# funkelab/cellulus

Hardware: AMD Instinct MI355X
Metric: train crops/sec (U-Net fwd+bwd + OCE loss + Adam) (higher is better)
Workload: dtype f32 (exact 3xbf16 operand split, 6 products, f32 accumulate)

## Files before the change

### cellulus_amd/_clx.py

```python

import ctypes
import os
from ctypes import POINTER, Structure, c_char_p, c_double, c_int, c_longlong, c_size_t, c_void_p

import torch

_HERE = os.path.dirname(os.path.abspath(__file__))
LIB_PATH = os.path.join(_HERE, "libclx.so")


class ClxError(RuntimeError):
    """A libclx entry point returned a negative status."""


class ClxSrc(Structure):

    _fields_ = [
        ("ptr", c_void_p),
        ("C", c_int),
        ("ld", c_int),
        ("D", c_int),
        ("H", c_int),
        ("W", c_int),
        ("oz", c_int),
# ... 52 lines not shown
        ("ld_pool", c_int),
        ("tile_list", c_void_p),
        ("tile_count", c_int),
        ("precision", c_int),
        ("wplanes", c_void_p),
        ("aplanes", c_void_p),
        ("aplanes_valid", c_int),
        ("dyplanes", c_void_p),
        ("dyplanes_valid", c_int),
        ("out_planes", c_void_p),
        ("out_colsum", c_void_p),
    ]


_P = c_void_p
_I = c_int
_LL = c_longlong
_D = c_double

PROTOTYPES = {
    "clx_last_error": (c_char_p, []),
    "clx_abi_version": (_I, []),
    "clx_device_count": (_I, []),
    "clx_profile_enable": (_I, [_I]),
    "clx_profile_read": (_I, [_I, POINTER(c_double), POINTER(c_double), POINTER(c_double)]),
    "clx_profile_clock": (_I, [POINTER(c_double), POINTER(c_double), _I]),
    "clx_conv_fwd": (_I, [POINTER(ClxConvDesc), _P]),
    "clx_conv_wgrad": (_I, [POINTER(ClxConvDesc), _P, _I, _P, _P, _P]),
    "clx_chain64_fwd": (_I, [_P, _I, _LL, _P, _P, _P, _I, _P, _I, _P, _P, _I, _I, _P, _I, _P, _I, _P]),
    "clx_chain64_bwd": (_I, [_P, _I, _I, _P, _I, _P, _I, _I, _LL, _P, _P, _P, _I, _P, _P, _P, _P, _P]),
    "clx_pack_weights": (_I, [_P, _P, _I, _I, _I, _I, _I, _I, _P]),
    "clx_pack_weights_batch": (_I, [_P, _I, _LL, _P]),
    "clx_unpack_wgrad": (_I, [_P, _P, _I, _I, _I, _I, _I, _P]),
    "clx_unpack_wgrad_wino": (_I, [_P, _P, _I, _I, _I, _I, _I, _I, _I, _P]),
    "clx_conv_workspace_bytes": (c_size_t, [POINTER(ClxConvDesc), _I]),
    "clx_conv_vcache_bytes": (c_size_t, [POINTER(ClxConvDesc), _I]),
    "clx_conv_sp_covers": (_I, [POINTER(ClxConvDesc), _I]),
    "clx_planes_bytes": (c_size_t, [_LL, _I]),
    "clx_split_planes": (_I, [_P, _LL, _LL, _I, _P, _P]),
    "clx_join_planes": (_I, [_P, _LL, _I, _P, _LL, _P]),
    "clx_gemm_planes": (_I, [_P, _P, _I, _I, _I, _P, _I, _P, _I, _P]),
    "clx_wgrad_planes": (_I, [_P, _P, _LL, _I, _I, _P, _I, _P]),
    "clx_conv_fused_applicable": (_I, [POINTER(ClxConvDesc)]),
    "clx_conv_fused_workspace_bytes": (c_size_t, [POINTER(ClxConvDesc)]),
    "clx_planar_to_pixel": (_I, [_P, _P, _I, _I, _LL, _I, _P]),
    "clx_pixel_to_planar": (_I, [_P, _P, _I, _I, _LL, _I, _P]),
# ... 169 lines not shown
```

### cellulus_amd/csrc/clx_common.h

```cpp
#pragma once
#include <hip/hip_runtime.h>
#include <hip/hip_ext.h>
#include <stdint.h>
#include <stdio.h>
#include <stdarg.h>
#include "../../include/clx.h"

void clx_set_error(const char* fmt, ...);

#define CLX_REQUIRE(cond, ...)                \
  do {                                        \
    if (!(cond)) {                            \
      clx_set_error(__VA_ARGS__);             \
      return CLX_ERR_ARG;                     \
    }                                         \
  } while (0)

#define CLX_CHECK_LAUNCH(name)                                           \
  do {                                                                   \
    hipError_t e__ = hipGetLastError();                                  \
    if (e__ != hipSuccess) {                                             \
      clx_set_error("%s: launch failed: %s", name, hipGetErrorString(e__)); \
      return CLX_ERR_LAUNCH;                                             \
    }                                                                    \
// ... 7 lines not shown
};
static inline FastDiv make_fastdiv(uint32_t d) {
  FastDiv f;
  f.d = d;
  uint32_t l = 0;
  while ((1ull << l) < d) ++l;
  f.l = l;
  f.m = (uint32_t)(((1ull << 32) * ((1ull << l) - d)) / d + 1);
  return f;
}
__device__ __forceinline__ uint32_t fdiv(uint32_t n, const FastDiv& f) {
  return (__umulhi(f.m, n) + n) >> f.l;
}

__device__ __forceinline__ int xcd_remap(int bid, int nblocks) {
  const int q = nblocks >> 3, r = nblocks & 7;
  const int xcd = bid & 7, idx = bid >> 3;
  const int base = (xcd < r) ? xcd * (q + 1) : r * (q + 1) + (xcd - r) * q;
  return base + idx;
}

static inline int cdiv(long long a, long long b) { return (int)((a + b - 1) / b); }

int clx_conv_validate(const clx_conv_desc* d, const char* who);

bool clx_smallc_applicable(const clx_conv_desc* d);
int clx_smallc_fwd(const clx_conv_desc* d, hipStream_t st);
int clx_smallc_wgrad(const clx_conv_desc* d, const float* dy, int ld_dy, float* dwpack,
                     float* dbias, hipStream_t st);

int clx_igemm_launch(const clx_conv_desc* d, int batch, long long bs_in, long long bs_w,
                     long long bs_out, hipStream_t st);
int clx_wgrad_launch(const clx_conv_desc* d, const float* dy, int ld_dy, float* dwpack, float* dbias,
                     int batch, long long bs_x, long long bs_dy, long long bs_out, hipStream_t st);
bool clx_sp_fwd_rule(const clx_conv_desc* d);
bool clx_sp_wgrad_rule(const clx_conv_desc* d);
bool clx_sp_applicable(const clx_conv_desc* d);
bool clx_wino_sp(const clx_conv_desc* d);
int clx_sp_launch(const void* A, const void* B, int M, int N, int K, long long rows_a, int batch, long long bs_a, long long bs_b,
                  long long bs_out, const clx_conv_desc* ep, hipStream_t st);
int clx_sp_clock_read(double* shader_ticks, double* wall_ticks, int reset);
int clx_sp_split(const float* x, long long ld, long long rows, int K, void* planes, float* colsum, int nreal, hipStream_t st);
int clx_sp_wgrad_launch(const void* dy_planes, const void* x_planes, long long rows, int N, int C, int batch, long long bs_dy,
                        long long bs_x, long long bs_out, float* dw, int ld_dw, hipStream_t st);
int clx_wino_fwd(const clx_conv_desc* d, hipStream_t st);
int clx_wino_wgrad(const clx_conv_desc* d, const float* dy, int ld_dy, float* dwpack, float* dbias,
// ... 17 lines not shown
```

### cellulus_amd/csrc/clx_core.hip

```cpp
#include "clx_common.h"

static thread_local char g_err[512] = "";

void clx_set_error(const char* fmt, ...) {
  va_list ap;
  va_start(ap, fmt);
  vsnprintf(g_err, sizeof(g_err), fmt, ap);
  va_end(ap);
}

extern "C" const char* clx_last_error(void) { return g_err; }
extern "C" int clx_abi_version(void) { return 13; }
extern "C" int clx_device_count(void) {
  int n = 0;
  if (hipGetDeviceCount(&n) != hipSuccess) {
    (void)hipGetLastError();
    return 0;
  }
  return n;
}

#include <vector>

namespace {
struct ProfRec { int kind; double flops; hipEvent_t e0, e1; };
bool g_prof_on = false;
std::vector<ProfRec> g_prof;
}

bool clx_prof_enabled() { return g_prof_on; }

void clx_prof_events(int kind, double flops, hipEvent_t* e0, hipEvent_t* e1) {
  *e0 = *e1 = nullptr;
  ProfRec r;
  r.kind = kind; r.flops = flops;
  if (hipEventCreate(&r.e0) != hipSuccess) return;
  if (hipEventCreate(&r.e1) != hipSuccess) { (void)hipEventDestroy(r.e0); return; }
  g_prof.push_back(r);
  *e0 = r.e0; *e1 = r.e1;
}

extern "C" int clx_profile_enable(int on) {
  g_prof_on = on != 0;
// ... 20 lines not shown
```

### cellulus_amd/csrc/conv_smallc.hip

```cpp
#include "clx_common.h"

namespace {

struct SmallP {
  const float* x;
  int ld_x, B, D, H, W;
  int oz, oy, ox;
  int ID, IH, IW, KD, KH, KW, PD, PH, PW, OD, OH, OW;
  int N, M, taps;
  FastDiv dOW, dOH, dOD;
  const float* wpack;
  const float* bias;
  float* out;
  int ld_out, relu;
  const float* dy;
  int ld_dy;
  float* dwp;
  float* dbias;
  int tiles_per_block;
  int RX, items;
  FastDiv dRX;
};

constexpr int PT = 64;
// ... 388 lines not shown
    f32x4 acc = bv;
#pragma unroll
    for (int rr = 0; rr < R; ++rr)
#pragma unroll
      for (int tx = 0; tx < 3; ++tx) acc += xv[rr * 3 + tx] * w[rr * 3 + tx];
    if (relu) {
#pragma unroll
      for (int e = 0; e < 4; ++e) acc[e] = fmaxf(acc[e], 0.f);
    }
    if (live && live_n) *reinterpret_cast<f32x4*>(out + (size_t)r * ld_out + nn) = acc;
  }
}

bool grey_applicable(const clx_conv_desc* d, int ld_act) {
  return d->c_real == 1 && d->KH == 3 && d->KW == 3 && (d->KD == 1 || d->KD == 3) && d->PD == 0 &&
         d->PH == 0 && d->PW == 0 && d->N % 4 == 0 && ld_act % 4 == 0;
}

dim3 grey_grid(SmallP& p) {
  p.RX = cdiv(p.OW, 4);
  p.items = p.B * p.OD * p.OH * p.RX;
  p.dRX = make_fastdiv(p.RX);
  const int ny = cdiv(p.N, 64);
  int nx = 768 / ny;
  if (nx < 1) nx = 1;
  if (nx > cdiv(p.items, 4)) nx = cdiv(p.items, 4);
  return dim3(nx, ny);
}

bool fill(const clx_conv_desc* d, SmallP& p) {
  const clx_src& S = d->src[0];
  p.x = S.ptr; p.ld_x = S.ld; p.B = d->B; p.D = S.D; p.H = S.H; p.W = S.W;
  p.oz = S.oz; p.oy = S.oy; p.ox = S.ox;
  p.ID = d->ID; p.IH = d->IH; p.IW = d->IW;
  p.KD = d->KD; p.KH = d->KH; p.KW = d->KW;
  p.PD = d->PD; p.PH = d->PH; p.PW = d->PW;
  p.OD = d->ID + 2 * d->PD - d->KD + 1;
  p.OH = d->IH + 2 * d->PH - d->KH + 1;
  p.OW = d->IW + 2 * d->PW - d->KW + 1;
  p.N = d->N;
  p.M = d->B * p.OD * p.OH * p.OW;
  p.taps = d->KD * d->KH * d->KW;
  p.dOW = make_fastdiv(p.OW); p.dOH = make_fastdiv(p.OH); p.dOD = make_fastdiv(p.OD);
  return true;
}

int pick_ng(int N) {
  int ng = 4;
  while (ng < 64 && ng * 4 < N) ng *= 2;
  return ng;
// ... 85 lines not shown
```

### cellulus_amd/csrc/gemm_sp.hip

```cpp
#include "clx_common.h"
#include "sp_planes.h"
#include <stdlib.h>
#include <type_traits>

__device__ unsigned long long g_sp_clk_ticks[2];
int clx_sp_clock_read(double* shader_ticks, double* wall_ticks, int reset) {
  unsigned long long h[2] = {0ull, 0ull};
  if (hipMemcpyFromSymbol(h, HIP_SYMBOL(g_sp_clk_ticks), sizeof(h)) != hipSuccess) return CLX_ERR_LAUNCH;
  *shader_ticks = (double)h[0];
  *wall_ticks = (double)h[1];
  if (reset) {
    const unsigned long long z[2] = {0ull, 0ull};
    if (hipMemcpyToSymbol(HIP_SYMBOL(g_sp_clk_ticks), z, sizeof(z)) != hipSuccess) return CLX_ERR_LAUNCH;
  }
  return CLX_OK;
}

namespace {

typedef __bf16 bf16x8 __attribute__((ext_vector_type(8)));
using sp::u32x2;
using sp::u32x4;
using sp::FRAG;
using sp::KSTEP;
// ... 959 lines not shown
  }
  return cache[dev];
}

int clx_sp_zero_tail(void* planes, long long rows, int K, int batch, long long bs, hipStream_t st) {
  if (sp::padded_rows(rows) == rows || batch <= 0) return CLX_OK;
  const int ksteps = K / 16;
  const long long total = (sp::padded_rows(rows) / 32 - rows / 32) * ksteps * 6 * 32;
  sp_zero_tail_kernel<<<dim3((unsigned)cdiv(total, 256), (unsigned)batch), 256, 0, st>>>((char*)planes, bs, rows, ksteps);
  return CLX_OK;
}

extern "C" size_t clx_planes_bytes(long long rows, int K) {
  if (rows <= 0 || K <= 0 || K % 16 != 0) return 0;
  return (size_t)sp::planes_bytes(rows, K);
}

int clx_sp_split(const float* x, long long ld, long long rows, int K, void* planes, float* colsum, int nreal, hipStream_t st) {
  CLX_REQUIRE(x != nullptr && planes != nullptr, "clx_split_planes: null pointer");
  CLX_REQUIRE(rows > 0 && K > 0 && K % 16 == 0 && ld >= K && ld % 4 == 0, "clx_split_planes: K must be a multiple of 16, ld >= K a multiple of 4");
  CLX_REQUIRE(((uintptr_t)x & 15) == 0 && ((uintptr_t)planes & 15) == 0, "clx_split_planes: pointers must be 16-byte aligned");
  const int ksteps = K / 16;
  const long long nfrag = sp::padded_rows(rows) / 32 * ksteps;
  long long blocks = (nfrag + 3) / 4;
  if (blocks > 8192) blocks = 8192;
  if (colsum != nullptr) {
    if (blocks > 2048) blocks = 2048;
    int g = ksteps % 4 == 0 ? 4 : ksteps % 2 == 0 ? 2 : 1;
    const long long unit = ksteps / g;
    blocks = (blocks + unit - 1) / unit * unit;
    CLX_LAUNCH_KIND(CLX_PROF_SPLIT_PLANES, sp_split_kernel<true>, dim3((unsigned)blocks), dim3(256), 0, st, x, ld, rows, ksteps, (char*)planes,
                    nfrag, colsum, nreal);
  } else {
    CLX_LAUNCH_KIND(CLX_PROF_SPLIT_PLANES, sp_split_kernel<false>, dim3((unsigned)blocks), dim3(256), 0, st, x, ld, rows, ksteps, (char*)planes,
                    nfrag, (float*)nullptr, 0);
  }
  return CLX_OK;
}

extern "C" int clx_split_planes(const float* x, long long ld, long long rows, int K, void* planes, clx_stream stream) {
  const int rc = clx_sp_split(x, ld, rows, K, planes, nullptr, 0, (hipStream_t)stream);
  if (rc) return rc;
  CLX_CHECK_LAUNCH("clx_split_planes");
  return CLX_OK;
}

extern "C" int clx_join_planes(const void* planes, long long rows, int K, float* x, long long ld, clx_stream stream) {
  CLX_REQUIRE(x != nullptr && planes != nullptr, "clx_join_planes: null pointer");
  CLX_REQUIRE(rows > 0 && K > 0 && K % 16 == 0 && ld >= K, "clx_join_planes: K must be a multiple of 16, ld >= K");
  const long long nfrag = sp::padded_rows(rows) / 32 * (K / 16);
  long long blocks = (nfrag + 3) / 4;
  if (blocks > 8192) blocks = 8192;
  sp_join_kernel<<<dim3((unsigned)blocks), dim3(256), 0, (hipStream_t)stream>>>((const char*)planes, ld, rows, K / 16, x, nfrag);
  CLX_CHECK_LAUNCH("clx_join_planes");
  return CLX_OK;
}
// ... 126 lines not shown
```

### cellulus_amd/csrc/glue.hip

```cpp
#include "clx_common.h"

namespace {

inline int grid_for(long long total, int block) {
  long long g = (total + block - 1) / block;
  if (g > 8192) g = 8192;
  if (g < 1) g = 1;
  return (int)g;
}

struct Dec {
  FastDiv c4, w, h, d;
};
inline Dec make_dec(int C4, int W, int H, int D) {
  return Dec{make_fastdiv((uint32_t)C4), make_fastdiv((uint32_t)W), make_fastdiv((uint32_t)H), make_fastdiv((uint32_t)D)};
}
__device__ __forceinline__ void decode(uint32_t i, const Dec& dc, uint32_t& pixel, int& c4, int& x, int& y, int& z, int& b) {
  pixel = fdiv(i, dc.c4);
  c4 = (int)(i - pixel * dc.c4.d);
  const uint32_t q1 = fdiv(pixel, dc.w);
  x = (int)(pixel - q1 * dc.w.d);
  const uint32_t q2 = fdiv(q1, dc.h);
  y = (int)(q1 - q2 * dc.h.d);
  const uint32_t q3 = fdiv(q2, dc.d);
  z = (int)(q2 - q3 * dc.d.d);
  b = (int)q3;
}

__device__ __forceinline__ f32x4 ld4(const float* p) { return *reinterpret_cast<const f32x4*>(p); }
__device__ __forceinline__ void st4(float* p, f32x4 v) { *reinterpret_cast<f32x4*>(p) = v; }

__global__ void maxpool_fwd_kernel(const float* __restrict__ x, float* __restrict__ y,
// ... 434 lines not shown
    noise_inject_kernel<1><<<grid_for((long long)T * n, 256), 256, 0, st>>>(rnd, raw, out, T, n_half, n, p);
  CLX_CHECK_LAUNCH("clx_noise_inject");
  return CLX_OK;
}

extern "C" int clx_zero_many(void* const* buffers, const long long* nbytes, int count, clx_stream stream) {
  CLX_REQUIRE(count >= 0 && (count == 0 || (buffers && nbytes)), "clx_zero_many: bad arguments");
  hipStream_t st = (hipStream_t)stream;
  for (int first = 0; first < count; first += 8) {
    ZeroManyP p;
    p.count = 0;
    p.first16[0] = 0;
    for (int k = first; k < count && k < first + 8; ++k) {
      CLX_REQUIRE(nbytes[k] >= 0 && nbytes[k] % 4 == 0, "clx_zero_many: sizes are multiples of 4 bytes");
      if (nbytes[k] == 0) continue;
      CLX_REQUIRE(buffers[k] && ((uintptr_t)buffers[k] & 15) == 0, "clx_zero_many: buffers are 16-byte aligned");
      const int q = p.count++;
      p.base[q] = (unsigned long long)(uintptr_t)buffers[k];
      p.first16[q + 1] = p.first16[q] + (unsigned long long)nbytes[k] / 16;
      p.tail_words[q] = (unsigned int)(nbytes[k] % 16) / 4;
    }
    if (p.count == 0) continue;
    for (int q = p.count; q < 8; ++q) { p.base[q] = 0; p.first16[q + 1] = p.first16[p.count]; p.tail_words[q] = 0; }
    long long g = (long long)((p.first16[p.count] + 255) / 256);
    g = g < 1 ? 1 : (g > 4096 ? 4096 : g);
    zero_many_kernel<<<(int)g, 256, 0, st>>>(p);
  }
  CLX_CHECK_LAUNCH("clx_zero_many");
  return CLX_OK;
}

extern "C" int clx_gather_rows_f64(const double* src, const int* rows, long long n, int width, double* dst,
                                   clx_stream stream) {
  CLX_REQUIRE(n >= 0 && width > 0 && (n == 0 || (src && rows && dst)), "clx_gather_rows_f64: bad arguments");
  if (n == 0) return CLX_OK;
  gather_rows_f64_kernel<<<grid_for(n * width, 256), 256, 0, (hipStream_t)stream>>>(src, rows, n, width, dst);
  CLX_CHECK_LAUNCH("clx_gather_rows_f64");
  return CLX_OK;
}

static int subpixel_launch(bool to_space, const float* src, float* dst, int ld_lo, int ld_hi, int B,
                           int D, int H, int W, int N, int fz, int fy, int fx, hipStream_t st,
                           const char* who) {
  CLX_REQUIRE(src && dst, "%s: null pointer", who);
  CLX_REQUIRE(B > 0 && D > 0 && H > 0 && W > 0 && N > 0 && N % 4 == 0, "%s: bad extents", who);
  CLX_REQUIRE(fz >= 1 && fy >= 1 && fx >= 1, "%s: bad factors", who);
  CLX_REQUIRE(ld_lo % 4 == 0 && ld_lo >= fz * fy * fx * N && ld_hi % 4 == 0 && ld_hi >= N, "%s: bad strides", who);
  const long long total = (long long)B * D * H * W * fz * fy * fx * (N / 4);
  if (to_space)
// ... 84 lines not shown
```

### cellulus_amd/csrc/pack.hip

```cpp
#include "clx_common.h"

namespace {

__global__ void pack_weights_kernel(const float* __restrict__ w, float* __restrict__ wp,
                                    int cout, int cin, int taps, int cin_pad,
                                    int cout_pad, int mode, long long total) {
  for (long long i = (long long)blockIdx.x * blockDim.x + threadIdx.x; i < total;
       i += (long long)gridDim.x * blockDim.x) {
    float v = 0.f;
    if (mode == CLX_PACK_FWD) {
      const int c = (int)(i % cin_pad);
      const long long t = i / cin_pad;
      const int tap = (int)(t % taps);
      const int n = (int)(t / taps);
      if (c < cin) v = w[((long long)n * cin + c) * taps + tap];
    } else {
      const int n = (int)(i % cout_pad);
      const long long t = i / cout_pad;
      const int tap = (int)(t % taps);
      const int c = (int)(t / taps);
      if (n < cout && c < cin) v = w[((long long)n * cin + c) * taps + (taps - 1 - tap)];
    }
    wp[i] = v;
  }
// ... 85 lines not shown
  for (long long i = (long long)blockIdx.x * blockDim.x + threadIdx.x; i < total;
       i += (long long)gridDim.x * blockDim.x) {
    const int tap = (int)(i % taps);
    const long long t = i / taps;
    const int c = (int)(t % g.cin), n = (int)(t / g.cin);
    if (c < g.C0) {
      gw[i] = g_skip[((long long)n * g.C0 + c) * taps + tap];
      continue;
    }
    const int d = tap / (g.k[1] * g.k[2]), h = (tap / g.k[2]) % g.k[1], x = tap % g.k[2];
    float v = 0.f;
    for (int a0 = 0; a0 < g.f[0]; ++a0)
      for (int a1 = 0; a1 < g.f[1]; ++a1)
        for (int a2 = 0; a2 < g.f[2]; ++a2) {
          const int ph = (a0 * g.f[1] + a1) * g.f[2] + a2;
          const int zt = (sp_low_tap(g.f[0], a0, d) * g.zk[1] + sp_low_tap(g.f[1], a1, h)) * g.zk[2] +
                         sp_low_tap(g.f[2], a2, x);
          v += g_eff[(((long long)ph * g.N + n) * g.C1 + (c - g.C0)) * ztaps + zt];
        }
    gw[i] = v;
  }
}

inline int grid_for(long long total, int block) {
  long long g = (total + block - 1) / block;
  if (g > 4096) g = 4096;
  if (g < 1) g = 1;
  return (int)g;
}

}

extern "C" int clx_pack_weights(const float* w, float* wp, int cout, int cin, int taps,
                                int cin_pad, int cout_pad, int mode, clx_stream stream) {
  CLX_REQUIRE(w && wp, "clx_pack_weights: null pointer");
  CLX_REQUIRE(cout > 0 && cin > 0 && taps > 0, "clx_pack_weights: bad extents");
  CLX_REQUIRE(cin_pad >= cin && cout_pad >= cout && cin_pad % 4 == 0 && cout_pad % 4 == 0,
              "clx_pack_weights: padded extents must be >= real and multiples of 4");
  if (mode == CLX_PACK_WINO4_ADJOINT) {
    CLX_REQUIRE(taps == 9 || taps == 27, "clx_pack_weights: the adjoint form exists for 3x3 and 3x3x3 kernels");
    clx_wino_pack(w, wp, cout, cin, cin_pad, cout_pad, 2, 4, 3, taps == 27 ? 3 : 1, (hipStream_t)stream);
    CLX_CHECK_LAUNCH("clx_pack_weights(winograd adjoint)");
    return CLX_OK;
  }
  if (mode == CLX_PACK_WINO4_FUSED) {
    CLX_REQUIRE((taps == 9 || taps == 4) && cout_pad % 64 == 0 && cin_pad % 8 == 0,
                "clx_pack_weights: the fused Winograd layout exists for 2-D 3x3 / 2x2 kernels with cout_pad %% 64 == 0 and "
                "cin_pad %% 8 == 0");
    clx_wino_pack(w, wp, cout, cin, cin_pad, cout_pad, 3, 4, taps == 9 ? 3 : 2, 1, (hipStream_t)stream);
    CLX_CHECK_LAUNCH("clx_pack_weights(winograd fused)");
    return CLX_OK;
  }
// ... 94 lines not shown
```

### cellulus_amd/csrc/wino.hip

```cpp
#include "clx_common.h"
#include "sp_planes.h"
#include "wino_tables.h"

namespace {

inline int grid_for(long long total, int block) {
  long long g = (total + block - 1) / block;
  if (g > 16384) g = 16384;
  if (g < 1) g = 1;
  return (int)g;
}

__device__ __forceinline__ f32x4 ld4(const float* p) { return *reinterpret_cast<const f32x4*>(p); }
__device__ __forceinline__ void st4(float* p, f32x4 v) { *reinterpret_cast<f32x4*>(p) = v; }

struct Geom {
  int B, SH, SW, oy, ox;
  int ID, SD, oz;
  int IH, IW, P;
  int OH, OW, th, tw;
  long long T;
};

template <int MT, int R, bool PL = false>
__global__ __launch_bounds__(256) void wino_input_kernel(const float* __restrict__ x, int ld_x, int C4, Geom g,
                                                         float* __restrict__ V, long long total,
                                                         const int* __restrict__ tile_list = nullptr, long long Tc = 0,
                                                         long long plane_bytes = 0) {
  using W = WT<MT, R>;
  constexpr int A = W::A;
  const int C = C4 * 4;
  const long long Trows = tile_list ? Tc : g.T;
  const long long plane = Trows * C;
  for (long long i = (long long)blockIdx.x * blockDim.x + threadIdx.x; i < total;
// ... 147 lines not shown
        } else {
          for (int e = 0; e < 4 && n + e < Nreal; ++e) {
            float xv = v[e];
            if (mask) xv = (mask[m * ld_mask + n + e] > 0.f) ? xv : 0.f;
            out[m * ld_out + n + e] = xv;
          }
        }
        if (pool_out) {
          if ((a & 1) == 0 && (cc & 1) == 0) pm[a >> 1][cc >> 1] = v;
          else {
#pragma unroll
            for (int e = 0; e < 4; ++e) pm[a >> 1][cc >> 1][e] = fmaxf(pm[a >> 1][cc >> 1][e], v[e]);
          }
          if ((a & 1) && (cc & 1)) {
            const long long pm_ = ((long long)b * (g.OH >> 1) + (oy >> 1)) * (g.OW >> 1) + (ox >> 1);
            st4(pool_out + pm_ * ld_pool + n, pm[a >> 1][cc >> 1]);
          }
        }
      }
    }
  }
}

constexpr int ADJ_SEG = 8;

__global__ __launch_bounds__(256) void wino_adjoint_output_kernel(const float* __restrict__ Pm, int C4, int Bn, int th,
                                                                  int tw, int IH, int IW, const float* __restrict__ mask,
                                                                  int ld_mask, const unsigned int* __restrict__ mask_bits,
                                                                  int ld_mask_bits, float* __restrict__ out, int ld_out,
                                                                  int Creal, long long total) {
  using W = WT<4, 3>;
  constexpr int A = 6;
  const int C = C4 * 4;
  const int bh = (IH + 3) / 4, bw = (IW + 3) / 4;
  const int nseg = (bh + ADJ_SEG - 1) / ADJ_SEG;
  const long long plane = (long long)Bn * th * tw * C;
  for (long long i = (long long)blockIdx.x * blockDim.x + threadIdx.x; i < total;
       i += (long long)gridDim.x * blockDim.x) {
    const int c = (int)(i % C4) * 4;
    long long t = i / C4;
    const int bx = (int)(t % bw);
    long long q = t / bw;
    const int sg = (int)(q % nseg);
    const int b = (int)(q / nseg);
    const int by0 = sg * ADJ_SEG, by1 = min(by0 + ADJ_SEG, bh);
    f32x4 carry[2][4];
#pragma unroll
    for (int a = 0; a < 2; ++a)
#pragma unroll
      for (int e = 0; e < 4; ++e) carry[a][e] = f32x4{0.f, 0.f, 0.f, 0.f};
    for (int ty = by0 - 1; ty < by1; ++ty) {
      f32x4 d[A][4];
#pragma unroll
      for (int a = 0; a < A; ++a)
#pragma unroll
        for (int e = 0; e < 4; ++e) d[a][e] = f32x4{0.f, 0.f, 0.f, 0.f};
      if (ty >= 0 && ty < th) {
#pragma unroll
        for (int ux = 0; ux < 2; ++ux) {
          const int tx = bx - ux;
          if (tx < 0 || tx >= tw) continue;
          const float* src = Pm + (((long long)b * th + ty) * tw + tx) * C + c;
#pragma unroll
          for (int s2 = 0; s2 < A; ++s2) {
            f32x4 pcol[A], wcol[A];
#pragma unroll
            for (int r = 0; r < A; ++r) pcol[r] = ld4(src + (r * A + s2) * plane);
#pragma unroll
            for (int a = 0; a < A; ++a) {
              f32x4 v = {0.f, 0.f, 0.f, 0.f};
              bool first = true;
#pragma unroll
              for (int r = 0; r < A; ++r) axpy(v, first, W::BT[r][a], pcol[r]);
              wcol[a] = v;
            }
#pragma unroll
            for (int e = 0; e < 4; ++e) {
              if (ux && e >= 2) continue;
              const float coef = ux ? W::BT[s2][4 + (e & 1)] : W::BT[s2][e];
#pragma unroll
              for (int a = 0; a < A; ++a) {
                bool first = false;
                axpy(d[a][e], first, coef, wcol[a]);
              }
            }
          }
        }
      }
      if (ty >= by0) {
#pragma unroll
        for (int a = 0; a < 4; ++a) {
          const int y = 4 * ty + a;
          if (y >= IH) continue;
#pragma unroll
          for (int e = 0; e < 4; ++e) {
            const int x = 4 * bx + e;
            if (x >= IW) continue;
            f32x4 v = d[a][e];
            if (a < 2) v += carry[a][e];
            const long long m = ((long long)b * IH + y) * IW + x;
            if (mask_bits) {
              const unsigned int wbits = mask_bits[m * ld_mask_bits + (c >> 5)] >> (c & 31);
#pragma unroll
              for (int k = 0; k < 4; ++k) v[k] = ((wbits >> k) & 1u) ? v[k] : 0.f;
            }
            if (c + 3 < Creal) {
              if (mask) {
                const f32x4 mk = ld4(mask + m * ld_mask + c);
#pragma unroll
                for (int k = 0; k < 4; ++k) v[k] = (mk[k] > 0.f) ? v[k] : 0.f;
              }
              st4(out + m * ld_out + c, v);
            } else {
              for (int k = 0; k < 4 && c + k < Creal; ++k) {
                float xv = v[k];
                if (mask) xv = (mask[m * ld_mask + c + k] > 0.f) ? xv : 0.f;
                out[m * ld_out + c + k] = xv;
              }
            }
          }
        }
      }
#pragma unroll
      for (int e = 0; e < 4; ++e) { carry[0][e] = d[4][e]; carry[1][e] = d[5][e]; }
    }
  }
}

template <int MT, int R, bool PL = false>
__global__ __launch_bounds__(256) void wino_dy_kernel(const float* __restrict__ dy, int ld_dy, int N4,
                                                      Geom g, float* __restrict__ Md,
                                                      float* __restrict__ dbias, int Nreal,
                                                      long long total, long long plane_bytes = 0) {
  using W = WT<MT, R>;
  constexpr int A = W::A;
  extern __shared__ float bacc[];
  const int N = N4 * 4;
  const long long plane = g.T * N;
  if (dbias) {
    for (int k = threadIdx.x; k < N; k += blockDim.x) bacc[k] = 0.f;
    __syncthreads();
  }
  for (long long i = (long long)blockIdx.x * blockDim.x + threadIdx.x; i < total;
       i += (long long)gridDim.x * blockDim.x) {
    int n;
    long long t;
    if constexpr (PL) {
// ... 442 lines not shown
      int rc = clx_sp_zero_tail(V, gin.T, C, AA, pbV, st);
      if (rc) return rc;
      CLX_LAUNCH_KIND(CLX_PROF_WINO_TRANSFORM, (wino_input_kernel<MT, R, true>), dim3(grid_for(tot_in, 256)), dim3(256), 0, st, S.ptr, S.ld, C / 4,
                      gin, V, tot_in, (const int*)nullptr, 0ll, pbV);
    } else {
      const long long tot_in = gin.T * (C / 4);
      CLX_LAUNCH_KIND(CLX_PROF_WINO_TRANSFORM, (wino_input_kernel<MT, R>), dim3(grid_for(tot_in, 256)), dim3(256), 0, st, S.ptr, S.ld, C / 4, gin, V,
                      tot_in, (const int*)nullptr, 0ll, 0ll);
    }
  }
  if (spx) {
    const int rc = clx_sp_zero_tail(Md, gout.T, N, AA, pbM, st);
    if (rc) return rc;
  }
  if (d->dy_vcache) {
    Geom gd = gout;
    gd.SH = gout.OH; gd.SW = gout.OW; gd.oy = gd.ox = 0;
    gd.ID = gd.SD = out_planes(d); gd.oz = 0;
    gd.IH = gout.OH; gd.IW = gout.OW; gd.P = R - 1;
    gd.OH = gout.OH + R - 1; gd.OW = gout.OW + R - 1;
    gd.th = (gd.OH + MT - 1) / MT; gd.tw = (gd.OW + MT - 1) / MT;
    gd.T = (long long)gd.B * gd.th * gd.tw;
    const long long tot = spx ? sp_items(gd.T, N) : gd.T * (N / 4);
    int blocks = grid_for(tot, 256);
    if (dbias && blocks > 2048) blocks = 2048;
    if (spx) {
      const long long pbD = sp::planes_bytes(gd.T, N);
      const int rc = clx_sp_zero_tail(d->dy_vcache, gd.T, N, AA, pbD, st);
      if (rc) return rc;
      CLX_LAUNCH_KIND(CLX_PROF_WINO_TRANSFORM, (wino_dy_dual_kernel<MT, R, true>), dim3(blocks), dim3(256), (size_t)N * sizeof(float), st, dy, ld_dy,
                      N / 4, gd, gout, (float*)d->dy_vcache, Md, dbias, N, tot, pbD, pbM);
    } else {
      CLX_LAUNCH_KIND(CLX_PROF_WINO_TRANSFORM, (wino_dy_dual_kernel<MT, R>), dim3(blocks), dim3(256), (size_t)N * sizeof(float), st, dy, ld_dy, N / 4,
                      gd, gout, (float*)d->dy_vcache, Md, dbias, N, tot, 0ll, 0ll);
    }
  } else {
    const long long tot_dy = spx ? sp_items(gout.T, N) : gout.T * (N / 4);
    int blocks = grid_for(tot_dy, 256);
    if (blocks > 2048) blocks = 2048;
    if (spx)
      CLX_LAUNCH_KIND(CLX_PROF_WINO_TRANSFORM, (wino_dy_kernel<MT, R, true>), dim3(blocks), dim3(256), (size_t)N * sizeof(float), st, dy, ld_dy, N / 4,
                      gout, Md, dbias, N, tot_dy, pbM);
    else
      CLX_LAUNCH_KIND(CLX_PROF_WINO_TRANSFORM, (wino_dy_kernel<MT, R>), dim3(blocks), dim3(256), (size_t)N * sizeof(float), st, dy, ld_dy, N / 4, gout,
                      Md, dbias, N, tot_dy, 0ll);
  }
  if (spx) {
    CLX_REQUIRE(gin.T == gout.T, "clx_conv_wgrad(winograd): tile counts of input and output differ");
    CLX_REQUIRE(d->det_turns == nullptr, "clx_conv_wgrad: the reproducible mode exists for the float32 precision only");
    const int rc = clx_sp_wgrad_launch(Md, V, gin.T, N, C, AA, pbM, pbV, (long long)N * C, dwpack, C, st);
    if (rc) return rc;
    CLX_CHECK_LAUNCH("clx_conv_wgrad(winograd, split precision)");
    return CLX_OK;
  }
  clx_conv_desc gd = gemm_desc(V, C, d, gin);
  gd.N = N;
  gd.det_turns = d->det_turns;
  const int rc = clx_wgrad_launch(&gd, Md, N, dwpack, nullptr, AA, gin.T * C, gout.T * N,
                                  (long long)d->KD * N * C, st);
  if (rc) return rc;
  CLX_CHECK_LAUNCH("clx_conv_wgrad(winograd)");
  return CLX_OK;
// ... 52 lines not shown
  float* P = (float*)d->workspace;
  float* Mdy = P + (size_t)36 * Tdx * Cp;
  if (spx) {
    CLX_REQUIRE(d->wplanes != nullptr, "clx_conv_fwd(adjoint): precision f32x3bf16 needs wplanes");
    const char* Mp = (const char*)d->workspace + 36 * sp::planes_bytes(Tdx, Cp);
    clx_conv_desc ep = {};
    ep.out = P; ep.ld_out = Cp;
    const int rc = clx_sp_launch(Mp, d->wplanes, (int)Tdy, Cp, Nf, Tdy, 36, sp::planes_bytes(Tdy, Nf), sp::planes_bytes(Cp, Nf),
                                 Tdx * Cp, &ep, st);
    if (rc) return rc;
  } else {
  clx_conv_desc gd = {};
  gd.nsrc = 1;
  gd.src[0].ptr = Mdy; gd.src[0].C = Nf; gd.src[0].ld = Nf;
  gd.src[0].D = planes_dy; gd.src[0].H = 1; gd.src[0].W = th * tw;
  gd.src[0].fz = gd.src[0].fy = gd.src[0].fx = 1;
  gd.B = d->B; gd.ID = planes_dy; gd.IH = 1; gd.IW = th * tw;
  gd.KD = d->KD; gd.KH = gd.KW = 1; gd.PD = d->PD;
  gd.N = Cp; gd.wpack = d->wpack; gd.out = P; gd.ld_out = Cp;
  const int rc = clx_igemm_launch(&gd, 36, Tdy * Nf, (long long)Cp * d->KD * Nf, Tdx * Cp, st);
  if (rc) return rc;
  }
  const int IH = OHf + 2, IW = OWf + 2;
  const int nseg = ((IH + 3) / 4 + ADJ_SEG - 1) / ADJ_SEG;
  const long long total = (long long)d->B * planes_dx * nseg * ((IW + 3) / 4) * (Cp / 4);
  CLX_LAUNCH_KIND(CLX_PROF_WINO_TRANSFORM, wino_adjoint_output_kernel, dim3(grid_for(total, 256)), dim3(256), 0, st, P, Cp / 4,
                  d->B * planes_dx, th, tw, IH, IW, d->mask, d->ld_mask, d->mask_bits, d->ld_mask_bits, d->out, d->ld_out, Cp, total);
  CLX_CHECK_LAUNCH("clx_conv_fwd(winograd adjoint)");
  return CLX_OK;
}

int clx_wino_fwd(const clx_conv_desc* d, hipStream_t st) {
  if (d->adjoint) return wino_adjoint(d, st);
  CLX_REQUIRE(applicable(d), "clx_conv_fwd: Winograd does not apply to this geometry");
  const size_t need = clx_conv_workspace_bytes(d, CLX_PASS_FWD);
  CLX_REQUIRE(d->workspace != nullptr && d->workspace_bytes >= need && need > 0,
              "clx_conv_fwd: Winograd needs %zu workspace bytes (%zu given)", need, d->workspace_bytes);
  CLX_REQUIRE(((uintptr_t)d->workspace & 15) == 0 && ((uintptr_t)d->vcache & 15) == 0,
              "clx_conv_fwd: workspace / vcache must be 16-byte aligned");
  if (d->KH == 2) return wino_fwd_t<4, 2>(d, st);
  return tile_of(d) == 4 ? wino_fwd_t<4, 3>(d, st) : wino_fwd_t<2, 3>(d, st);
}

int clx_wino_wgrad(const clx_conv_desc* d, const float* dy, int ld_dy, float* dwpack, float* dbias,
                   hipStream_t st) {
  CLX_REQUIRE(applicable(d) && d->PH == 0, "clx_conv_wgrad: Winograd does not apply to this geometry");
  const size_t need = clx_conv_workspace_bytes(d, CLX_PASS_WGRAD);
  CLX_REQUIRE(d->workspace != nullptr && d->workspace_bytes >= need && need > 0,
              "clx_conv_wgrad: Winograd needs %zu workspace bytes (%zu given)", need, d->workspace_bytes);
  CLX_REQUIRE(((uintptr_t)d->workspace & 15) == 0 && ((uintptr_t)d->vcache & 15) == 0,
// ... 47 lines not shown
```

### cellulus_amd/models/dual.py

```python

import os

import torch

from .. import _clx
from .plan import UNetPlan
from .topology import forward_flops


class _Rows:

    def __init__(self, parts, attr):
        self._parts, self._attr = parts, attr

    def __getitem__(self, name):
        return torch.cat([getattr(p, self._attr)[name] for p in self._parts], dim=0)

    def __contains__(self, name):
        return name in getattr(self._parts[0], self._attr)

    def __bool__(self):
        return bool(getattr(self._parts[0], self._attr))

    def get(self, name, default=None):
        return self[name] if name in self else default

    def keys(self):
        return getattr(self._parts[0], self._attr).keys()


def dual_stream_wanted(topo, batch, keep_activations):
    if not keep_activations or batch < 2 or batch % 2 or os.environ.get("CLX_STREAMS", "2") == "1":
        return False
    if os.environ.get("CLX_DETERMINISTIC", "0") == "1":
        return False
    return forward_flops(topo, batch // 2) >= float(os.environ.get("CLX_STREAMS_MIN_GFLOP", "100")) * 1e9


class DualPlan:

    def __init__(self, topo, batch, device, keep_activations):
        assert batch % 2 == 0 and keep_activations
        self.topo, self.B, self.device, self.keep = topo, int(batch), device, True
        self.parts = [UNetPlan(topo, batch // 2, device, True) for _ in range(2)]
        self.streams = [torch.cuda.Stream(device=device) for _ in range(2)]
        self._events = [[], [], []]
        self._shared = False
        self.buf = _Rows(self.parts, "buf")

    def __getattr__(self, name):
        if name in ("parts", "streams"):
# ... 9 lines not shown
            b._alloc_backward()
            b.share_from(a)
            self._shared = True
        b._packed_version = a._packed_version

    def _fork(self):
        main = torch.cuda.current_stream(self.device)
        for s in self.streams:
            s.wait_stream(main)
        return main

    def _join(self, main):
        for s in self.streams:
            main.wait_stream(s)

    def forward(self, raw, params, out=None):
        t = self.topo
        assert self._shared, "pack_weights(need_dgrad=True) must run before forward"
        raw = raw.contiguous()
        if out is None:
            out = torch.empty((self.B, t.out_channels) + tuple(t.out_shape[3 - t.nd:]), dtype=torch.float32,
                              device=self.device)
        h = self.B // 2
        main = self._fork()
        for i, (p, s) in enumerate(zip(self.parts, self.streams)):
            with torch.cuda.stream(s):
                p.forward(raw[i * h:(i + 1) * h], params, out=out[i * h:(i + 1) * h])
        self._join(main)
        return out

    def _event(self, i, k):
        ev = self._events[i]
        while len(ev) <= k:
            ev.append(torch.cuda.Event())
        return ev[k]

    def backward(self, dout, params, grads, on_layer_done=None, flat_grad=None, dx=None):
        dout = dout.contiguous()
        h = self.B // 2
        self.parts[0].zero_gradients(grads, flat_grad)
        main = self._fork()
        dxs = [dx[:h], dx[h:]] if dx is not None else [None, None]
        self._backward_halves([dout[:h], dout[h:]], params, grads, on_layer_done, main, dxs=dxs)
        self._join(main)

    def train_pass(self, raw, params, grads, flat_grad, loss_fn, after_loss=None, on_layer_done=None):
        t = self.topo
        assert self._shared, "pack_weights(need_dgrad=True) must run before train_pass"
        raw = raw.contiguous()
        out = torch.empty((self.B, t.out_channels) + tuple(t.out_shape[3 - t.nd:]), dtype=torch.float32,
                          device=self.device)
        h = self.B // 2
        main = self._fork()
        douts = []
        for i, (p, s) in enumerate(zip(self.parts, self.streams)):
            with torch.cuda.stream(s):
                o = p.forward(raw[i * h:(i + 1) * h], params, out=out[i * h:(i + 1) * h])
                douts.append(loss_fn(o, i * h, (i + 1) * h))
                self._event(i, 0).record(s)
        self.parts[0].zero_gradients(grads, flat_grad)
        zeroed = self._event(2, 0)
        zeroed.record(main)
        for i, s in enumerate(self.streams):
            main.wait_event(self._event(i, 0))
            s.wait_event(zeroed)
        if after_loss is not None:
            after_loss()
        self._backward_halves(douts, params, grads, on_layer_done, main)
        self._join(main)
        return out

    def _backward_halves(self, douts, params, grads, on_layer_done, main, dxs=(None, None)):
        st_main = _clx.stream_ptr(self.device)
        gens = []
        for p, s, d, dx in zip(self.parts, self.streams, douts, dxs):
# ... 24 lines not shown
```

### include/clx.h

```cpp
#ifndef CLX_H
#define CLX_H

#include <stddef.h>
#include <stdint.h>

#ifdef __cplusplus
extern "C" {
#endif

typedef void* clx_stream;

enum clx_status {
  CLX_OK = 0,
  CLX_ERR_ARG = -1,
  CLX_ERR_LAUNCH = -2,
  CLX_ERR_WORKSPACE = -3
};

const char* clx_last_error(void);
int clx_abi_version(void);
int clx_device_count(void);

enum clx_profile_kind {
  CLX_PROF_IGEMM_WIDE = 0,
  CLX_PROF_IGEMM_NARROW = 1,
  CLX_PROF_WGRAD = 2,
  CLX_PROF_GEMM_SP = 3,
  CLX_PROF_WGRAD_SP = 4,
  CLX_PROF_SPLIT_PLANES = 5,
  CLX_PROF_CHAIN64 = 6,
  CLX_PROF_MS_PREPARE = 7,
  CLX_PROF_MS_ASSIGN = 8,
  CLX_PROF_CC = 9,
  CLX_PROF_GROW_SHRINK = 10,
  CLX_PROF_MINMAX = 11,
  CLX_PROF_HISTOGRAM = 12,
  CLX_PROF_NOISE_STATS = 13,
  CLX_PROF_WINO_FUSED = 14,
  CLX_PROF_WINO_TRANSFORM = 15,
  CLX_PROF_GEMM_SP2 = 16
};
int clx_profile_enable(int on);
int clx_profile_read(int kind, double* launches, double* total_ms, double* total_flops);
int clx_profile_clock(double* shader_ticks, double* wall_ticks_100mhz, int reset);
// ... 326 lines not shown
```

Measured before the change: 310.3.

## Centralize grid sizing with stream-aware caps and restructure Winograd adjoint output kernel

Adds a shared grid-size helper with per-kernel caps that can bound block counts by a fraction of the CUs when two streams run concurrently, and wraps the dual-stream forward, backward and train paths to set that mode. Because every quarter constant is zero, the CU bound is effectively inactive, so grid sizes match the previous caps. Separately, the Winograd adjoint output kernel is rewritten so each block processes a column group across channels, computing the full 6x6 patch per tile and passing the overlapping columns to the neighbouring thread through shared memory. It also uses longer row segments when there is enough parallelism. The kernel rewrite aims to cut redundant loads and transforms of neighbouring tiles, at the cost of block-level syncs and extra registers.

```diff
diff --git a/cellulus_amd/_clx.py b/cellulus_amd/_clx.py
--- a/cellulus_amd/_clx.py
+++ b/cellulus_amd/_clx.py
@@ -98,6 +98,9 @@
     "clx_last_error": (c_char_p, []),
     "clx_abi_version": (_I, []),
     "clx_device_count": (_I, []),
+    "clx_set_concurrent_streams": (_I, [_I]),
+    "clx_stream_grid_blocks": (_I, [_LL, _I, _I, _I, _I]),
+    "clx_set_stream_grid_cus": (_I, [_I]),
     "clx_profile_enable": (_I, [_I]),
     "clx_profile_read": (_I, [_I, POINTER(c_double), POINTER(c_double), POINTER(c_double)]),
     "clx_profile_clock": (_I, [POINTER(c_double), POINTER(c_double), _I]),
diff --git a/cellulus_amd/csrc/clx_common.h b/cellulus_amd/csrc/clx_common.h
--- a/cellulus_amd/csrc/clx_common.h
+++ b/cellulus_amd/csrc/clx_common.h
@@ -53,6 +53,20 @@
 
 static inline int cdiv(long long a, long long b) { return (int)((a + b - 1) / b); }
 
+enum clx_stream_kind {
+  CLX_SG_TRANSFORM = 0,
+  CLX_SG_TRANSFORM_ACC,
+  CLX_SG_SPLIT,
+  CLX_SG_SPLIT_COLSUM,
+  CLX_SG_GLUE,
+  CLX_SG_PACK,
+  CLX_SG_FIRST,
+  CLX_SG_FILL,
+  CLX_SG_KINDS
+};
+#define CLX_SG_ARG(kind, n) ((kind) | ((n) << 8))
+int clx_stream_grid(long long total_items, int block, int kind);
+
 int clx_conv_validate(const clx_conv_desc* d, const char* who);
 
 bool clx_smallc_applicable(const clx_conv_desc* d);
diff --git a/cellulus_amd/csrc/clx_core.hip b/cellulus_amd/csrc/clx_core.hip
--- a/cellulus_amd/csrc/clx_core.hip
+++ b/cellulus_amd/csrc/clx_core.hip
@@ -19,6 +19,79 @@
   }
   return n;
 }
+
+#include <atomic>
+
+namespace {
+enum { SG_CLASS_TRANSFORM = 0, SG_CLASS_SPLIT, SG_CLASS_REST, SG_CLASSES };
+struct SgRule { int cap, cls; };
+constexpr SgRule SG_RULES[CLX_SG_KINDS] = {
+    {16384, SG_CLASS_TRANSFORM},
+    {2048, SG_CLASS_TRANSFORM},
+    {8192, SG_CLASS_SPLIT},
+    {2048, SG_CLASS_SPLIT},
+    {8192, SG_CLASS_REST},
+    {4096, SG_CLASS_REST},
+    {768, SG_CLASS_REST},
+    {4096, SG_CLASS_REST},
+};
+constexpr int SG_QUARTERS_TRANSFORM = 0, SG_QUARTERS_SPLIT = 0, SG_QUARTERS_REST = 0;
+constexpr int SG_QUARTERS[SG_CLASSES] = {SG_QUARTERS_TRANSFORM, SG_QUARTERS_SPLIT, SG_QUARTERS_REST};
+
+std::atomic<int> g_sg_streams{1};
+std::atomic<int> g_sg_cus_forced{0};
+
+int sg_device_cus() {
+  static const int cus = [] {
+    int dev = 0;
+    hipDeviceProp_t prop;
+    if (hipGetDevice(&dev) != hipSuccess || hipGetDeviceProperties(&prop, dev) != hipSuccess) {
+      (void)hipGetLastError();
+      return 0;
+    }
+    return prop.multiProcessorCount;
+  }();
+  const int forced = g_sg_cus_forced.load(std::memory_order_relaxed);
+  return forced > 0 ? forced : cus;
+}
+}
+
+namespace {
+int sg_blocks(long long total, int block, int kind, int cus, int mode, int least_quarters) {
+  const int k = kind & 0xff, arg = kind >> 8;
+  if (k < 0 || k >= CLX_SG_KINDS || block <= 0 || arg < 0) return 0;
+  long long cap = SG_RULES[k].cap, unit = 1;
+  if (k == CLX_SG_FIRST && arg > 1) cap = cap / arg > 0 ? cap / arg : 1;
+  if (k == CLX_SG_SPLIT_COLSUM && arg > 1)
+    unit = arg / (arg % 4 == 0 ? 4 : arg % 2 == 0 ? 2 : 1);
+  long long g = total > 0 ? (total + block - 1) / block : 1;
+  if (g > cap) g = cap;
+  if (g < 1) g = 1;
+  g = (g + unit - 1) / unit * unit;
+  int quarters = SG_QUARTERS[SG_RULES[k].cls];
+  if (quarters <= 0) quarters = least_quarters;
+  if (mode >= 2 && cus > 0 && quarters > 0) {
+    long long bound = (long long)quarters * cus / 4 / unit * unit;
+    if (bound < unit) bound = unit;
+    if (g > bound) g = bound;
+  }
+  return (int)g;
+}
+}
+
+extern "C" int clx_stream_grid_blocks(long long total, int block, int kind, int cus, int mode) {
+  return sg_blocks(total, block, kind, cus, mode, 0);
+}
+
+int clx_stream_grid(long long total_items, int block, int kind) {
+  const int mode = g_sg_streams.load(std::memory_order_relaxed);
+  if (mode < 2) return sg_blocks(total_items, block, kind, 0, mode, 0);
+  const bool forced = g_sg_cus_forced.load(std::memory_order_relaxed) > 0;
+  return sg_blocks(total_items, block, kind, sg_device_cus(), mode, forced ? 4 : 0);
+}
+
+extern "C" int clx_set_concurrent_streams(int n) { return g_sg_streams.exchange(n < 1 ? 1 : n); }
+extern "C" int clx_set_stream_grid_cus(int cus) { return g_sg_cus_forced.exchange(cus < 0 ? 0 : cus); }
 
 #include <vector>
 
diff --git a/cellulus_amd/csrc/conv_smallc.hip b/cellulus_amd/csrc/conv_smallc.hip
--- a/cellulus_amd/csrc/conv_smallc.hip
+++ b/cellulus_amd/csrc/conv_smallc.hip
@@ -434,10 +434,7 @@
   p.items = p.B * p.OD * p.OH * p.RX;
   p.dRX = make_fastdiv(p.RX);
   const int ny = cdiv(p.N, 64);
-  int nx = 768 / ny;
-  if (nx < 1) nx = 1;
-  if (nx > cdiv(p.items, 4)) nx = cdiv(p.items, 4);
-  return dim3(nx, ny);
+  return dim3(clx_stream_grid(p.items, 4, CLX_SG_ARG(CLX_SG_FIRST, ny)), ny);
 }
 
 bool fill(const clx_conv_desc* d, SmallP& p) {
diff --git a/cellulus_amd/csrc/gemm_sp.hip b/cellulus_amd/csrc/gemm_sp.hip
--- a/cellulus_amd/csrc/gemm_sp.hip
+++ b/cellulus_amd/csrc/gemm_sp.hip
@@ -1005,16 +1005,12 @@
   CLX_REQUIRE(((uintptr_t)x & 15) == 0 && ((uintptr_t)planes & 15) == 0, "clx_split_planes: pointers must be 16-byte aligned");
   const int ksteps = K / 16;
   const long long nfrag = sp::padded_rows(rows) / 32 * ksteps;
-  long long blocks = (nfrag + 3) / 4;
-  if (blocks > 8192) blocks = 8192;
   if (colsum != nullptr) {
-    if (blocks > 2048) blocks = 2048;
-    int g = ksteps % 4 == 0 ? 4 : ksteps % 2 == 0 ? 2 : 1;
-    const long long unit = ksteps / g;
-    blocks = (blocks + unit - 1) / unit * unit;
+    const int blocks = clx_stream_grid(nfrag, 4, CLX_SG_ARG(CLX_SG_SPLIT_COLSUM, ksteps));
     CLX_LAUNCH_KIND(CLX_PROF_SPLIT_PLANES, sp_split_kernel<true>, dim3((unsigned)blocks), dim3(256), 0, st, x, ld, rows, ksteps, (char*)planes,
                     nfrag, colsum, nreal);
   } else {
+    const int blocks = clx_stream_grid(nfrag, 4, CLX_SG_SPLIT);
     CLX_LAUNCH_KIND(CLX_PROF_SPLIT_PLANES, sp_split_kernel<false>, dim3((unsigned)blocks), dim3(256), 0, st, x, ld, rows, ksteps, (char*)planes,
                     nfrag, (float*)nullptr, 0);
   }
diff --git a/cellulus_amd/csrc/glue.hip b/cellulus_amd/csrc/glue.hip
--- a/cellulus_amd/csrc/glue.hip
+++ b/cellulus_amd/csrc/glue.hip
@@ -2,12 +2,7 @@
 
 namespace {
 
-inline int grid_for(long long total, int block) {
-  long long g = (total + block - 1) / block;
-  if (g > 8192) g = 8192;
-  if (g < 1) g = 1;
-  return (int)g;
-}
+inline int grid_for(long long total, int block) { return clx_stream_grid(total, block, CLX_SG_GLUE); }
 
 struct Dec {
   FastDiv c4, w, h, d;
@@ -488,9 +483,7 @@
     }
     if (p.count == 0) continue;
     for (int q = p.count; q < 8; ++q) { p.base[q] = 0; p.first16[q + 1] = p.first16[p.count]; p.tail_words[q] = 0; }
-    long long g = (long long)((p.first16[p.count] + 255) / 256);
-    g = g < 1 ? 1 : (g > 4096 ? 4096 : g);
-    zero_many_kernel<<<(int)g, 256, 0, st>>>(p);
+    zero_many_kernel<<<clx_stream_grid((long long)p.first16[p.count], 256, CLX_SG_FILL), 256, 0, st>>>(p);
   }
   CLX_CHECK_LAUNCH("clx_zero_many");
   return CLX_OK;
diff --git a/cellulus_amd/csrc/pack.hip b/cellulus_amd/csrc/pack.hip
--- a/cellulus_amd/csrc/pack.hip
+++ b/cellulus_amd/csrc/pack.hip
@@ -131,12 +131,7 @@
   }
 }
 
-inline int grid_for(long long total, int block) {
-  long long g = (total + block - 1) / block;
-  if (g > 4096) g = 4096;
-  if (g < 1) g = 1;
-  return (int)g;
-}
+inline int grid_for(long long total, int block) { return clx_stream_grid(total, block, CLX_SG_PACK); }
 
 }
 
diff --git a/cellulus_amd/csrc/wino.hip b/cellulus_amd/csrc/wino.hip
--- a/cellulus_amd/csrc/wino.hip
+++ b/cellulus_amd/csrc/wino.hip
@@ -4,12 +4,7 @@
 
 namespace {
 
-inline int grid_for(long long total, int block) {
-  long long g = (total + block - 1) / block;
-  if (g > 16384) g = 16384;
-  if (g < 1) g = 1;
-  return (int)g;
-}
+inline int grid_for(long long total, int block) { return clx_stream_grid(total, block, CLX_SG_TRANSFORM); }
 
 __device__ __forceinline__ f32x4 ld4(const float* p) { return *reinterpret_cast<const f32x4*>(p); }
 __device__ __forceinline__ void st4(float* p, f32x4 v) { *reinterpret_cast<f32x4*>(p) = v; }
@@ -203,72 +198,83 @@
   }
 }
 
-constexpr int ADJ_SEG = 8;
+constexpr int ADJ_SEG = 8, ADJ_SEG_LONG = 16;
+constexpr int ADJ_MIN_ITEMS = 1024;
+
+template <int E0, int NE, int LD>
+__device__ __forceinline__ void adjoint_patch(const float* __restrict__ src, long long plane, f32x4 (&d)[6][LD]) {
+  using W = WT<4, 3>;
+  constexpr int A = 6;
+#pragma unroll
+  for (int s2 = 0; s2 < A; ++s2) {
+    f32x4 pcol[A], wcol[A];
+#pragma unroll
+    for (int r = 0; r < A; ++r) pcol[r] = ld4(src + (r * A + s2) * plane);
+#pragma unroll
+    for (int a = 0; a < A; ++a) {
+      f32x4 v = {0.f, 0.f, 0.f, 0.f};
+      bool first = true;
+#pragma unroll
+      for (int r = 0; r < A; ++r) axpy(v, first, W::BT[r][a], pcol[r]);
+      wcol[a] = v;
+    }
+#pragma unroll
+    for (int e = 0; e < NE; ++e) {
+#pragma unroll
+      for (int a = 0; a < A; ++a) {
+        bool first = false;
+        axpy(d[a][e], first, W::BT[s2][E0 + e], wcol[a]);
+      }
+    }
+  }
+}
 
 __global__ __launch_bounds__(256) void wino_adjoint_output_kernel(const float* __restrict__ Pm, int C4, int Bn, int th,
                                                                   int tw, int IH, int IW, const float* __restrict__ mask,
                                                                   int ld_mask, const unsigned int* __restrict__ mask_bits,
                                                                   int ld_mask_bits, float* __restrict__ out, int ld_out,
-                                                                  int Creal, long long total) {
-  using W = WT<4, 3>;
+                                                                  int Creal, int CL, int G, int seg, long long nitems) {
   constexpr int A = 6;
+  __shared__ f32x4 xch[2 * A * 256];
   const int C = C4 * 4;
   const int bh = (IH + 3) / 4, bw = (IW + 3) / 4;
-  const int nseg = (bh + ADJ_SEG - 1) / ADJ_SEG;
+  const int nseg = (bh + seg - 1) / seg, ngrp = (bw + G - 1) / G, nchunk = (C4 + CL - 1) / CL;
   const long long plane = (long long)Bn * th * tw * C;
-  for (long long i = (long long)blockIdx.x * blockDim.x + threadIdx.x; i < total;
-       i += (long long)gridDim.x * blockDim.x) {
-    const int c = (int)(i % C4) * 4;
-    long long t = i / C4;
-    const int bx = (int)(t % bw);
-    long long q = t / bw;
+  const int tid = threadIdx.x;
+  const int g = tid / CL, l = tid - g * CL;
+  for (long long it = blockIdx.x; it < nitems; it += gridDim.x) {
+    const int chunk = (int)(it % nchunk);
+    long long t = it / nchunk;
+    const int grp = (int)(t % ngrp);
+    long long q = t / ngrp;
     const int sg = (int)(q % nseg);
     const int b = (int)(q / nseg);
-    const int by0 = sg * ADJ_SEG, by1 = min(by0 + ADJ_SEG, bh);
-    f32x4 carry[2][4];
-#pragma unroll
-    for (int a = 0; a < 2; ++a)
-#pragma unroll
-      for (int e = 0; e < 4; ++e) carry[a][e] = f32x4{0.f, 0.f, 0.f, 0.f};
+    const int bx = grp * G + g, c = (chunk * CL + l) * 4;
+    const bool active = g < G && bx < bw && c < C;
+    const int by0 = sg * seg, by1 = min(by0 + seg, bh);
+    f32x4 d[A][A];
+#pragma unroll
+    for (int a = 0; a < A; ++a)
+#pragma unroll
+      for (int e = 0; e < A; ++e) d[a][e] = f32x4{0.f, 0.f, 0.f, 0.f};
     for (int ty = by0 - 1; ty < by1; ++ty) {
-      f32x4 d[A][4];
-#pragma unroll
-      for (int a = 0; a < A; ++a)
-#pragma unroll
-        for (int e = 0; e < 4; ++e) d[a][e] = f32x4{0.f, 0.f, 0.f, 0.f};
-      if (ty >= 0 && ty < th) {
-#pragma unroll
-        for (int ux = 0; ux < 2; ++ux) {
-          const int tx = bx - ux;
-          if (tx < 0 || tx >= tw) continue;
-          const float* src = Pm + (((long long)b * th + ty) * tw + tx) * C + c;
-#pragma unroll
-          for (int s2 = 0; s2 < A; ++s2) {
-            f32x4 pcol[A], wcol[A];
-#pragma unroll
-            for (int r = 0; r < A; ++r) pcol[r] = ld4(src + (r * A + s2) * plane);
-#pragma unroll
-            for (int a = 0; a < A; ++a) {
-              f32x4 v = {0.f, 0.f, 0.f, 0.f};
-              bool first = true;
-#pragma unroll
-              for (int r = 0; r < A; ++r) axpy(v, first, W::BT[r][a], pcol[r]);
-              wcol[a] = v;
-            }
-#pragma unroll
-            for (int e = 0; e < 4; ++e) {
-              if (ux && e >= 2) continue;
-              const float coef = ux ? W::BT[s2][4 + (e & 1)] : W::BT[s2][e];
-#pragma unroll
-              for (int a = 0; a < A; ++a) {
-                bool first = false;
-                axpy(d[a][e], first, coef, wcol[a]);
-              }
-            }
-          }
-        }
-      }
-      if (ty >= by0) {
+      const bool tile_row = ty >= 0 && ty < th;
+      if (tile_row) {
+        const float* row = Pm + ((long long)b * th + ty) * tw * C + c;
+        if (active && bx < tw) {
+          adjoint_patch<0, 6, A>(row + (long long)bx * C, plane, d);
+#pragma unroll
+          for (int a = 0; a < A; ++a) { xch[(2 * a) * 256 + tid] = d[a][4]; xch[(2 * a + 1) * 256 + tid] = d[a][5]; }
+        }
+        if (active && g == 0 && bx > 0) adjoint_patch<4, 2, A>(row + (long long)(bx - 1) * C, plane, d);
+        __syncthreads();
+        if (active && g > 0) {
+#pragma unroll
+          for (int a = 0; a < A; ++a) { d[a][0] += xch[(2 * a) * 256 + tid - CL]; d[a][1] += xch[(2 * a + 1) * 256 + tid - CL]; }
+        }
+        __syncthreads();
+      }
+      if (ty >= by0 && active) {
 #pragma unroll
         for (int a = 0; a < 4; ++a) {
           const int y = 4 * ty + a;
@@ -278,7 +284,6 @@
             const int x = 4 * bx + e;
             if (x >= IW) continue;
             f32x4 v = d[a][e];
-            if (a < 2) v += carry[a][e];
             const long long m = ((long long)b * IH + y) * IW + x;
             if (mask_bits) {
               const unsigned int wbits = mask_bits[m * ld_mask_bits + (c >> 5)] >> (c & 31);
@@ -303,7 +308,9 @@
         }
       }
 #pragma unroll
-      for (int e = 0; e < 4; ++e) { carry[0][e] = d[4][e]; carry[1][e] = d[5][e]; }
+      for (int a = 0; a < A; ++a)
+#pragma unroll
+        for (int e = 0; e < A; ++e) d[a][e] = (a < 2 && e < 4) ? d[a + 4][e] : f32x4{0.f, 0.f, 0.f, 0.f};
     }
   }
 }
@@ -792,8 +799,7 @@
     gd.th = (gd.OH + MT - 1) / MT; gd.tw = (gd.OW + MT - 1) / MT;
     gd.T = (long long)gd.B * gd.th * gd.tw;
     const long long tot = spx ? sp_items(gd.T, N) : gd.T * (N / 4);
-    int blocks = grid_for(tot, 256);
-    if (dbias && blocks > 2048) blocks = 2048;
+    const int blocks = clx_stream_grid(tot, 256, dbias ? CLX_SG_TRANSFORM_ACC : CLX_SG_TRANSFORM);
     if (spx) {
       const long long pbD = sp::planes_bytes(gd.T, N);
       const int rc = clx_sp_zero_tail(d->dy_vcache, gd.T, N, AA, pbD, st);
@@ -806,8 +812,7 @@
     }
   } else {
     const long long tot_dy = spx ? sp_items(gout.T, N) : gout.T * (N / 4);
-    int blocks = grid_for(tot_dy, 256);
-    if (blocks > 2048) blocks = 2048;
+    const int blocks = clx_stream_grid(tot_dy, 256, CLX_SG_TRANSFORM_ACC);
     if (spx)
       CLX_LAUNCH_KIND(CLX_PROF_WINO_TRANSFORM, (wino_dy_kernel<MT, R, true>), dim3(blocks), dim3(256), (size_t)N * sizeof(float), st, dy, ld_dy, N / 4,
                       gout, Md, dbias, N, tot_dy, pbM);
@@ -906,10 +911,14 @@
   if (rc) return rc;
   }
   const int IH = OHf + 2, IW = OWf + 2;
-  const int nseg = ((IH + 3) / 4 + ADJ_SEG - 1) / ADJ_SEG;
-  const long long total = (long long)d->B * planes_dx * nseg * ((IW + 3) / 4) * (Cp / 4);
-  CLX_LAUNCH_KIND(CLX_PROF_WINO_TRANSFORM, wino_adjoint_output_kernel, dim3(grid_for(total, 256)), dim3(256), 0, st, P, Cp / 4,
-                  d->B * planes_dx, th, tw, IH, IW, d->mask, d->ld_mask, d->mask_bits, d->ld_mask_bits, d->out, d->ld_out, Cp, total);
+  const int C4 = Cp / 4, CL = C4 < 64 ? C4 : 64, G = 256 / CL;
+  const int bh = (IH + 3) / 4, bw = (IW + 3) / 4;
+  const long long cols = (long long)d->B * planes_dx * cdiv(bw, G) * cdiv(C4, CL);
+  const int seg = cols * cdiv(bh, ADJ_SEG_LONG) >= ADJ_MIN_ITEMS ? ADJ_SEG_LONG : ADJ_SEG;
+  const long long nitems = cols * cdiv(bh, seg);
+  CLX_LAUNCH_KIND(CLX_PROF_WINO_TRANSFORM, wino_adjoint_output_kernel, dim3(grid_for(nitems * 256, 256)), dim3(256), 0, st, P, C4,
+                  d->B * planes_dx, th, tw, IH, IW, d->mask, d->ld_mask, d->mask_bits, d->ld_mask_bits, d->out, d->ld_out, Cp, CL,
+                  G, seg, nitems);
   CLX_CHECK_LAUNCH("clx_conv_fwd(winograd adjoint)");
   return CLX_OK;
 }
diff --git a/cellulus_amd/models/dual.py b/cellulus_amd/models/dual.py
--- a/cellulus_amd/models/dual.py
+++ b/cellulus_amd/models/dual.py
@@ -1,4 +1,5 @@
 
+import contextlib
 import os
 
 import torch
@@ -27,6 +28,16 @@
 
     def keys(self):
         return getattr(self._parts[0], self._attr).keys()
+
+
+@contextlib.contextmanager
+def _two_streams():
+    lib = _clx.load()
+    previous = lib.clx_set_concurrent_streams(2)
+    try:
+        yield
+    finally:
+        lib.clx_set_concurrent_streams(previous)
 
 
 def dual_stream_wanted(topo, batch, keep_activations):
@@ -82,11 +93,12 @@
             out = torch.empty((self.B, t.out_channels) + tuple(t.out_shape[3 - t.nd:]), dtype=torch.float32,
                               device=self.device)
         h = self.B // 2
-        main = self._fork()
-        for i, (p, s) in enumerate(zip(self.parts, self.streams)):
-            with torch.cuda.stream(s):
-                p.forward(raw[i * h:(i + 1) * h], params, out=out[i * h:(i + 1) * h])
-        self._join(main)
+        with _two_streams():
+            main = self._fork()
+            for i, (p, s) in enumerate(zip(self.parts, self.streams)):
+                with torch.cuda.stream(s):
+                    p.forward(raw[i * h:(i + 1) * h], params, out=out[i * h:(i + 1) * h])
+            self._join(main)
         return out
 
     def _event(self, i, k):
@@ -101,8 +113,9 @@
         self.parts[0].zero_gradients(grads, flat_grad)
         main = self._fork()
         dxs = [dx[:h], dx[h:]] if dx is not None else [None, None]
-        self._backward_halves([dout[:h], dout[h:]], params, grads, on_layer_done, main, dxs=dxs)
-        self._join(main)
+        with _two_streams():
+            self._backward_halves([dout[:h], dout[h:]], params, grads, on_layer_done, main, dxs=dxs)
+            self._join(main)
 
     def train_pass(self, raw, params, grads, flat_grad, loss_fn, after_loss=None, on_layer_done=None):
         t = self.topo
@@ -111,6 +124,10 @@
         out = torch.empty((self.B, t.out_channels) + tuple(t.out_shape[3 - t.nd:]), dtype=torch.float32,
                           device=self.device)
         h = self.B // 2
+        with _two_streams():
+            return self._train_pass(raw, params, grads, flat_grad, loss_fn, after_loss, on_layer_done, out, h)
+
+    def _train_pass(self, raw, params, grads, flat_grad, loss_fn, after_loss, on_layer_done, out, h):
         main = self._fork()
         douts = []
         for i, (p, s) in enumerate(zip(self.parts, self.streams)):
diff --git a/include/clx.h b/include/clx.h
--- a/include/clx.h
+++ b/include/clx.h
@@ -20,6 +20,10 @@
 const char* clx_last_error(void);
 int clx_abi_version(void);
 int clx_device_count(void);
+
+int clx_set_concurrent_streams(int n);
+int clx_stream_grid_blocks(long long total, int block, int kind, int cus, int mode);
+int clx_set_stream_grid_cus(int cus);
 
 enum clx_profile_kind {
   CLX_PROF_IGEMM_WIDE = 0,
```

New measurement: 310.5 (median of 6 runs). No clear change (+0.1%).
